# EvolBioInf/andi

Hardware: AMD Instinct MI355X
Metric: genome-pairs/sec (ordered pairs, n^2-n) over the N x N anchor-distance loop (higher is better)
Workload: dtype u8

## Files before the change

### andi_amd/csrc/esa_build.hip

```cpp
#include "andi_dev.h"
#include "esa_build.h"
#include "scan.h"
#include "knobs.h"

#include <cstring>

#define CHECK_LAUNCH()                                                                             \
	do {                                                                                           \
		hipError_t e_ = hipGetLastError();                                                         \
		if (e_ != hipSuccess) return e_;                                                           \
	} while (0)

__global__ __launch_bounds__(256) void k_phi_scatter(const int32_t *__restrict__ SA,
													 int32_t *__restrict__ phi, int32_t n) {
	int32_t r = blockIdx.x * blockDim.x + threadIdx.x;
	if (r >= n) return;
	int32_t prev = r ? SA[r - 1] : -1;
	phi[SA[r]] = prev;
}

#define PLCP_CHUNK 32
__global__ __launch_bounds__(256) void k_plcp_chunks(const uint8_t *__restrict__ S,
													 int32_t *__restrict__ phi_plcp, int32_t n) {
	int64_t chunk = (int64_t)blockIdx.x * blockDim.x + threadIdx.x;
	int64_t t0 = chunk * PLCP_CHUNK;
	if (t0 >= n) return;
	int32_t t1 = (int32_t)((t0 + PLCP_CHUNK < n) ? t0 + PLCP_CHUNK : n);
	uint32_t h = 0;
	for (int32_t t = (int32_t)t0; t < t1; ++t) {
		int32_t prev = phi_plcp[t];
		if (prev < 0) {
			phi_plcp[t] = -1;
			continue;
		}
		g_u8p a = (g_u8p)S + prev + h, b = (g_u8p)S + t + h;
		for (;;) {
			uint64_t x = ld_u64_unaligned(a) ^ ld_u64_unaligned(b);
			if (x) {
				h += (uint32_t)(__builtin_ctzll(x) >> 3);
				break;
			}
			h += 8, a += 8, b += 8;
		}
		phi_plcp[t] = (int32_t)h;
		h = h ? h - 1 : 0;
	}
}

__global__ __launch_bounds__(256) void k_lcp_fvc(const uint8_t *__restrict__ S,
												 const int32_t *__restrict__ SA,
												 const int32_t *__restrict__ plcp,
												 int32_t *__restrict__ LCP, uint8_t *__restrict__ FVC,
												 int32_t n) {
	int32_t r = blockIdx.x * blockDim.x + threadIdx.x;
	if (r > n) return;
	if (r == n) {
		LCP[n] = -1;
		return;
	}
	int32_t sa = SA[r];
	int32_t l = r ? plcp[sa] : -1;
	LCP[r] = l;
	FVC[r] = S[sa + l];
}

__global__ __launch_bounds__(256) void k_min64(const int32_t *__restrict__ in, int32_t count,
											   int32_t *__restrict__ out) {
	int64_t gid = (int64_t)blockIdx.x * blockDim.x + threadIdx.x;
	int32_t v = gid < count ? in[gid] : INT32_MAX;
	for (int off = 32; off; off >>= 1) {
		int32_t o = __shfl_xor(v, off);
		v = o < v ? o : v;
	}
	if ((threadIdx.x & 63) == 0 && gid < count) out[gid >> 6] = v;
}

__device__ __forceinline__ int32_t nearest_left_le(const MinTree &t, int32_t q, int32_t v) {
	int32_t cur = q - 1;
	int lvl = 0;
	for (;;) {
		bool found = false;
		for (;;) {
			if (t.lv[lvl][cur] <= v) {
				found = true;
				break;
			}
			if ((cur & 63) == 0) break;
			--cur;
		}
		if (found) break;
		cur = (cur >> 6) - 1;
		++lvl;
	}
	while (lvl > 0) {
		--lvl;
		cur = (cur << 6) + 63;
		while (t.lv[lvl][cur] > v) --cur;
	}
	return cur;
}

__device__ __forceinline__ int32_t nearest_right_lt(const MinTree &t, int32_t q, int32_t v) {
	int32_t cur = q + 1;
	int lvl = 0;
	for (;;) {
		bool found = false;
		for (;;) {
			if (t.lv[lvl][cur] < v) {
				found = true;
				break;
			}
			if ((cur & 63) == 63) break;
			++cur;
		}
		if (found) break;
		cur = (cur >> 6) + 1;
		++lvl;
	}
	while (lvl > 0) {
		--lvl;
		cur = cur << 6;
		while (t.lv[lvl][cur] >= v) ++cur;
	}
	return cur;
}

__global__ __launch_bounds__(256) void k_child_table(MinTree t, int32_t *__restrict__ CLD,
													 int32_t n) {
	int64_t gid = (int64_t)blockIdx.x * blockDim.x + threadIdx.x;
	if (gid >= n) return;
	int32_t q = (int32_t)gid + 1;
	const int32_t *LCP = t.lv[0];
	int32_t v = LCP[q];
	int32_t a = nearest_left_le(t, q, v);
	int32_t la = LCP[a];
	if (la == v) {
		CLD[a] = q;
		return;
	}
	int32_t b = nearest_right_lt(t, q, v);
	if (la <= LCP[b]) {
		CLD[b - 1] = q;
	} else {
		CLD[a] = q;
	}
}

__global__ __launch_bounds__(256) void k_kmer_table(EsaDev Ed, int4 *__restrict__ tab,
													int32_t *__restrict__ flags) {
	uint32_t code = blockIdx.x * blockDim.x + threadIdx.x;
	if (code >= (1u << (2 * ANDI_CACHE_K))) return;
	const EsaG E = esa_global(Ed);
	auto sym = [&](int pos) { return code_nt(code >> (2 * (ANDI_CACHE_K - 1 - pos))); };

	Ival in = esa_root(E);
	int pos = 0;
	Ival out;
	for (;;) {
		if (pos >= ANDI_CACHE_K) {
			out = in;
			break;
		}
		Ival ij = esa_child(E, in, sym(pos));
		if (ival_empty(ij)) {
			out = in;
			break;
		}
		if (ij.i == ij.j) {
			ij.l = pos + 1;
			out = ij;
			break;
		}
		if (ij.l <= pos + 1) {
			in = ij;
			++pos;
			continue;
		}
		if (ij.l >= ANDI_CACHE_K) {
			out = in;
			break;
		}
		g_u8p suf = E.S + E.SA[ij.i];
		int k = pos + 1;
		bool decided = false;
		for (; k < ij.l; ++k) {
			uint8_t e = suf[k];
			if (!is_acgt(e)) {
				out = ij;
				decided = true;
				flags[2] = 1;
				break;
			}
			if (e != sym(k)) {
				out = in;
				decided = true;
				break;
			}
		}
		if (decided) break;
		in = ij;
		pos = ij.l;
	}
	tab[code] = make_int4(out.l, out.i, out.j, out.m);
}

#define REC_V(x) ((x)&15u)
#define REC_SEP(x) (((x) >> 4) & 3u)
#define REC_CODE(x) ((x) >> 6)

__device__ __forceinline__ uint32_t suffix_rec(const uint8_t *__restrict__ N0, const int32_t *__restrict__ SA,
											   int32_t r, int K) {
	const uint32_t p = (uint32_t)SA[r];
	const uint64_t w = ld_u64_unaligned((g_u8p)N0 + (p >> 1)) >> (4 * (p & 1u));
	const uint64_t stop = (w & 0x4444444444444444ull) | (1ull << 62);
	uint32_t v = (uint32_t)__builtin_ctzll(stop) >> 2;
	uint32_t sep = 0;
	if (v < (uint32_t)K) {
		const uint32_t c = (uint32_t)(w >> (4 * v)) & 7u;
		sep = c == 4 ? 1u : (c == 5 ? 2u : 3u);
	} else {
		v = (uint32_t)K;
	}
	auto squeeze = [](uint32_t x) {
		x &= 0x33333333u;
		x = (x | (x >> 2)) & 0x0f0f0f0fu;
		x = (x | (x >> 4)) & 0x00ff00ffu;
		x = (x | (x >> 8)) & 0x0000ffffu;
		return x;
	};
	uint32_t y = __brev(squeeze((uint32_t)w) | (squeeze((uint32_t)(w >> 32)) << 16));
	y = ((y & 0x55555555u) << 1) | ((y >> 1) & 0x55555555u);
	return ((y >> (32 - 2 * K)) << 6) | (sep << 4) | v;
}

__device__ __forceinline__ uint32_t rec_lcp(uint32_t a, uint32_t b, int K) {
	uint32_t x = REC_CODE(a) ^ REC_CODE(b);
	uint32_t same = x ? (uint32_t)(__builtin_clz(x) - (32 - 2 * K)) >> 1 : (uint32_t)K;
	uint32_t va = REC_V(a), vb = REC_V(b);
	uint32_t m = va < vb ? va : vb;
	return same < m ? same : m;
}

__device__ __forceinline__ uint32_t rec_lcp_code(uint32_t code, uint32_t a, int K) {
	uint32_t x = code ^ REC_CODE(a);
	uint32_t same = x ? (uint32_t)(__builtin_clz(x) - (32 - 2 * K)) >> 1 : (uint32_t)K;
	uint32_t va = REC_V(a);
	return same < va ? same : va;
}

#ifndef PT_BLOCK
#define PT_BLOCK 256
#endif
#ifndef PT_GAPS
#define PT_GAPS 3
#endif
#define PT_TILE (PT_BLOCK * PT_GAPS)
#define PT_WORDS (PT_TILE / 64)
#define PT_RANKED 4096
__device__ __forceinline__ uint32_t wave_scan_incl(uint32_t v) {
	v += (uint32_t)__builtin_amdgcn_update_dpp(0, (int)v, 0x111, 0xf, 0xf, false);
	v += (uint32_t)__builtin_amdgcn_update_dpp(0, (int)v, 0x112, 0xf, 0xf, false);
	v += (uint32_t)__builtin_amdgcn_update_dpp(0, (int)v, 0x114, 0xf, 0xf, false);
	v += (uint32_t)__builtin_amdgcn_update_dpp(0, (int)v, 0x118, 0xf, 0xf, false);
	v += (uint32_t)__builtin_amdgcn_update_dpp(0, (int)v, 0x142, 0xa, 0xf, false);
	v += (uint32_t)__builtin_amdgcn_update_dpp(0, (int)v, 0x143, 0xc, 0xf, false);
	return v;
}

__device__ __forceinline__ uint32_t first_code(bool has, uint32_t L, int K) {
	const uint32_t v = REC_V(L), sh = 2 * ((uint32_t)K - v);
	const uint32_t c = ((REC_CODE(L) >> sh) << sh) + (v == (uint32_t)K ? 1u : 0u);
	return has ? c : 0u;
}

__device__ __forceinline__ void probe_table_block(const uint8_t *__restrict__ N0, const int32_t *__restrict__ SA,
												  const uint32_t *__restrict__ REC, const uint16_t *__restrict__ REC2, uint2 *__restrict__ deep,
												  int32_t *__restrict__ flags, int32_t n, int K, int single_ext, uint32_t block) {
	__shared__ uint32_t s_first[PT_TILE];
	__shared__ uint32_t s_absent[PT_TILE];
	__shared__ uint32_t s_h[PT_TILE + 2];
	__shared__ uint2 s_present[PT_TILE];
	__shared__ uint32_t s_rec[PT_TILE + 5];
	__shared__ uint64_t s_some[PT_WORDS];
	__shared__ uint32_t s_bits[PT_RANKED / 32];
	__shared__ uint32_t s_before[PT_RANKED / 32];
	__shared__ uint16_t s_owner[PT_TILE];

	const uint32_t r0 = block * PT_TILE;
	const uint32_t lane = threadIdx.x & 63u, wave = threadIdx.x >> 6;
	auto make_rec = [&](int32_t j) { return REC ? REC[j] : suffix_rec(N0, SA, j, K); };
	uint32_t mine2[PT_GAPS];
	{
		uint32_t mine[PT_GAPS];
#pragma unroll
		for (int u = 0; u < PT_GAPS; ++u) {
			const uint32_t g = r0 + threadIdx.x + u * PT_BLOCK;
			mine[u] = g < (uint32_t)n ? make_rec((int32_t)g) : 0u;
			mine2[u] = (single_ext == 2 && REC2 && g < (uint32_t)n) ? REC2[g] : 0u;
		}
#pragma unroll
		for (int u = 0; u < PT_GAPS; ++u) s_rec[threadIdx.x + u * PT_BLOCK + 2] = mine[u];
	}
	if (threadIdx.x < 2) s_rec[threadIdx.x] = r0 + threadIdx.x >= 2 ? make_rec((int32_t)(r0 + threadIdx.x - 2)) : 0u;
	if (threadIdx.x == 2) s_rec[PT_TILE + 2] = r0 + PT_TILE < (uint32_t)n ? make_rec((int32_t)(r0 + PT_TILE)) : 0u;
	if (threadIdx.x < PT_RANKED / 32) s_bits[threadIdx.x] = 0;
	__syncthreads();
	auto rec = [&](int32_t j) {
		const uint32_t k = (uint32_t)j - r0 + 2;
		return k < PT_TILE + 3 ? s_rec[k] : make_rec(j);
	};
	const uint32_t full = (uint32_t)K;
	if (threadIdx.x == 0) s_h[0] = r0 >= 2 ? rec_lcp(s_rec[0], s_rec[1], K) : 0u;
	if (threadIdx.x == 1) s_h[PT_TILE + 1] = r0 + PT_TILE < (uint32_t)n ? rec_lcp(s_rec[PT_TILE + 1], s_rec[PT_TILE + 2], K) : 0u;

	uint32_t counts[PT_GAPS], firsts[PT_GAPS];
#pragma unroll
	for (int u = 0; u < PT_GAPS; ++u) {
		const uint32_t i = threadIdx.x + u * PT_BLOCK;
		const uint32_t gid = r0 + i;
		const bool live = gid <= (uint32_t)n;
		const int32_t r = (int32_t)(live ? gid : 0);
		const bool hasL = live && r > 0, hasR = live && r < n;
		const uint32_t Lr = s_rec[i + 1], Rr = s_rec[i + 2], a1 = s_rec[i + 3], a2 = s_rec[i + 4], a3 = s_rec[i + 5];
		const uint32_t L = hasL ? Lr : 0u, R = hasR ? Rr : 0u;
		const uint32_t sa_r = hasR ? (uint32_t)SA[r] : 0u;
		const uint32_t h = (hasL && hasR) ? rec_lcp(L, R, K) : 0u;
		s_h[i + 1] = h;
		uint32_t absent = 0, first = 1u << (2 * K), owns_present = 0;
		uint2 present = make_uint2(0, 0);

		if (live) {
			if (hasR && REC_V(R) == full && !(hasL && L == R)) {
				const bool in_tile = i + 5 < PT_TILE + 3;
				const int32_t m = a1 != R ? 0 : (a2 != R ? 1 : (a3 != R ? 2 : 3));
				int32_t j = in_tile ? r + m : r;
				const bool more = !in_tile || m == 3;
				if (more) {
					while (j + 1 < n && j - r < 16 && rec(j + 1) == R) ++j;
					if (j - r == 16 && j + 1 < n && rec(j + 1) == R) {
						int32_t lo = j + 1, hi = n - 1;
						while (lo < hi) {
							const int32_t mid = lo + ((hi - lo + 1) >> 1);
							if (rec(mid) == R) lo = mid; else hi = mid - 1;
						}
						j = lo;
					}
				}
				if (j == r) {
					const uint32_t pos = sa_r, e0 = pos + full;
					if (single_ext == 2 && REC2) {
						const uint32_t w = mine2[u];
						present = make_uint2(pos, DEEP_SINGLE | ((w >> 8) << 2) | ((w & 0xffu) << 6));
					} else if (single_ext != 1) {
						present = make_uint2(pos, DEEP_SINGLE | (1u << 2) | (full << 8));
					} else {
						const uint64_t w = ld_u64_unaligned((g_u8p)N0 + (e0 >> 1)) >> (4 * (e0 & 1u));
						uint32_t nval = (uint32_t)__builtin_ctzll((w & 0x4444444444444444ull) | (1ull << 52)) >> 2;
						auto squeeze = [](uint32_t x) {
							x &= 0x33333333u;
							x = (x | (x >> 2)) & 0x0f0f0f0fu;
							x = (x | (x >> 4)) & 0x00ff00ffu;
							x = (x | (x >> 8)) & 0x0000ffffu;
							return x;
						};
						const uint32_t ext = (squeeze((uint32_t)w) | (squeeze((uint32_t)(w >> 32)) << 16)) & ((1u << (2 * nval)) - 1u);
						present = make_uint2(pos, DEEP_SINGLE | (nval << 2) | (ext << 6));
					}
				} else {
					const bool fits = (uint32_t)(j - r) < (1u << 24);
					present = make_uint2(fits ? (uint32_t)r : 0u, fits ? DEEP_MULTI | ((uint32_t)(j - r) << 8) : (uint32_t)DEEP_SEARCH);
				}
				owns_present = 1;
			}

			if (__builtin_amdgcn_ballot_w64(hasR && (REC_SEP(R) == 1 || REC_SEP(R) == 2)) != 0 && hasR) {
				uint32_t k = REC_V(R), sp = REC_SEP(R);
				if (k >= 1 && k <= 8 && k < full && (sp == 1 || sp == 2) && (!hasL || h < k)) {
					int32_t j = r;
					while (j + 1 < n) {
						uint32_t X = rec(j + 1);
						if (REC_V(X) == k && REC_SEP(X) == sp && rec_lcp(R, X, K) == k) ++j; else break;
					}
					if (j > r && (j + 1 == n || rec_lcp(R, rec(j + 1), K) < k)) flags[0] = 1;
				}
			}

			const int32_t lo = (int32_t)first_code(hasL, L, K);
			const uint32_t shR = 2 * (full - REC_V(R));
			const int32_t hi = hasR ? (int32_t)((REC_CODE(R) >> shR) << shR) - 1 : (int32_t)((1u << (2 * K)) - 1u);
			if (lo <= hi) absent = (uint32_t)(hi - lo + 1);
			first = (uint32_t)lo;
		}
		s_first[i] = first, s_absent[i] = absent, s_present[i] = present;
		counts[u] = absent + owns_present, firsts[u] = first;
		const uint64_t b = __ballot(counts[u] != 0);
		if (lane == 0) s_some[u * (PT_BLOCK / 64) + wave] = b;
	}

	__syncthreads();
	const uint32_t base = first_code(r0 > 0, s_rec[1], K);
	const uint32_t total = (r0 + PT_TILE <= (uint32_t)n ? first_code(true, s_rec[PT_TILE + 1], K) : (1u << (2 * K))) - base;
	uint32_t owners_before;
	{
		const uint32_t mine = lane < PT_WORDS ? (uint32_t)__builtin_popcountll(s_some[lane]) : 0u;
		owners_before = wave_scan_incl(mine) - mine;
	}
#pragma unroll
	for (int u = 0; u < PT_GAPS; ++u) {
		const uint32_t word = u * (PT_BLOCK / 64) + wave;
		const uint32_t before = (uint32_t)__builtin_amdgcn_readlane((int)owners_before, __builtin_amdgcn_readfirstlane((int)word));
		if (counts[u] == 0) continue;
		const uint32_t i = threadIdx.x + u * PT_BLOCK, off = firsts[u] - base;
		s_owner[before + (uint32_t)__builtin_popcountll(s_some[word] & ((1ull << lane) - 1ull))] = (uint16_t)i;
		if (off < PT_RANKED) atomicOr(&s_bits[off >> 5], 1u << (off & 31u));
	}
	__syncthreads();
	if (wave == 0) {
		uint32_t carry = 0;
		for (uint32_t w0 = 0; w0 < PT_RANKED / 32; w0 += 64) {
			const uint32_t mine = (uint32_t)__builtin_popcount(s_bits[w0 + lane]), incl = wave_scan_incl(mine);
			s_before[w0 + lane] = carry + incl - mine;
			carry += (uint32_t)__builtin_amdgcn_readlane((int)incl, 63);
		}
	}
	__syncthreads();

	auto write_entry = [&](uint32_t t, uint32_t a) {
		const uint32_t c = base + t;
		const bool is_present = c - s_first[a] >= s_absent[a];
		const uint2 pres = s_present[a];
		const uint32_t rr = r0 + a;
		const bool gL = rr > 0, gR = rr < (uint32_t)n;
		const uint32_t gl = s_rec[a + 1], gr = s_rec[a + 2], hll = s_h[a], hrr = s_h[a + 2];
		const uint32_t xL = rec_lcp_code(c, gl, K), xR = rec_lcp_code(c, gr, K);
		const uint32_t lL = gL ? xL : 0u, lR = gR ? xR : 0u;
		const bool left = lL > lR, right = lR > lL;
		const uint32_t l = left ? lL : lR;
		const uint32_t idx = left ? rr - 1 : (right ? rr : 0u);
		const bool alone = left ? (rr < 2 || hll < l) : (rr + 1 >= (uint32_t)n || hrr < l);
		const uint32_t uniq = ((left || right) && l != 0) ? (alone ? 1u : 0u) : (n == 1 ? 1u : 0u);
		const uint2 val = is_present ? pres : make_uint2(idx, DEEP_FINAL | (uniq << 2) | (l << 8));
		__builtin_nontemporal_store(((unsigned long long)val.y << 32) | val.x, (unsigned long long *)(deep + c));
	};
	const uint32_t ranked = total < PT_RANKED ? total : PT_RANKED;
	for (uint32_t t = threadIdx.x; t < ranked; t += PT_BLOCK) {
		const uint32_t word = t >> 5;
		write_entry(t, s_owner[s_before[word] + (uint32_t)__builtin_popcount(s_bits[word] & (0xffffffffu >> (31u - (t & 31u)))) - 1u]);
	}
	for (uint32_t t = PT_RANKED + threadIdx.x; t < total; t += PT_BLOCK) {
		const uint32_t c = base + t;
		uint32_t a = 0, b = PT_TILE;
		while (b - a > 1) {
			const uint32_t mid = (a + b) >> 1;
			if (s_first[mid] <= c) a = mid; else b = mid;
		}
		write_entry(t, a);
	}
}

__global__ __launch_bounds__(PT_BLOCK) void k_probe_table(const uint8_t *__restrict__ N0, const int32_t *__restrict__ SA,
														  const uint32_t *__restrict__ rec, const uint16_t *__restrict__ rec2, uint2 *__restrict__ deep,
														  int32_t *__restrict__ flags, int32_t n, int K, int single_ext) {
	probe_table_block(N0, SA, rec, rec2, deep, flags, n, K, single_ext, blockIdx.x);
}

__global__ __launch_bounds__(PT_BLOCK) void k_probe_table_batch(const AndiIndexBatchItem *__restrict__ items) {
	const AndiIndexBatchItem it = items[blockIdx.y];
	if ((uint64_t)blockIdx.x * PT_TILE > (uint64_t)it.n) return;
	probe_table_block(it.N0, it.SA, it.rec, it.rec2, it.deep, it.flags, it.n, it.deepK, it.single_ext, blockIdx.x);
}

size_t andi_min_tree_entries(int32_t n) {
	size_t total = 0;
	size_t cnt = (size_t)n + 1;
	while (cnt > 64) {
		cnt = (cnt + 63) / 64;
		total += cnt;
	}
	return total ? total : 1;
}

int andi_index_single_ext(size_t queries, bool sorted_on_device) {
	const int coop = andi_coop_enabled();
	if (coop == 0) return 0;
	if (const char *f = andi_knob(KNOB_SINGLE_EXT)) {
		const int v = atoi(f);
		if (v >= 0 && v <= 2 && (v != 2 || sorted_on_device)) return v;
	}
	if (sorted_on_device) return 2;
	return (coop > 0 || queries >= 256) ? 1 : 0;
}

hipError_t andi_launch_index_build(const EsaBuildArgs &a, int single_ext, hipStream_t st) {
	const int32_t n = a.n;
	hipError_t e;
	e = andi_launch_pack_symbols(a.S, (size_t)n + 1 + 64, a.N0, a.N1, a.flags + 1, st);
	if (e != hipSuccess) return e;
	if (a.P) e = andi_launch_pack_planes(a.N0, (size_t)n + 1 + 64, a.P, st);
	if (e != hipSuccess) return e;
	k_probe_table<<<(unsigned)(((int64_t)n + 1 + PT_TILE - 1) / PT_TILE), PT_BLOCK, 0, st>>>(a.N0, a.SA, a.rec, a.rec2, a.deep, a.flags, n,
																				  a.deepK, single_ext);
	CHECK_LAUNCH();
	return hipSuccess;
}

hipError_t andi_launch_index_build_batch(const AndiIndexBatchItem *d_items, uint32_t count, int32_t max_n, hipStream_t st) {
	if (count == 0) return hipSuccess;
	hipError_t e = andi_launch_pack_symbols_batch(d_items, count, (size_t)max_n + 1 + 64, st);
	if (e != hipSuccess) return e;
	e = andi_launch_pack_planes_batch(d_items, count, (size_t)max_n, st);
	if (e != hipSuccess) return e;
	const dim3 grid((unsigned)(((int64_t)max_n + 1 + PT_TILE - 1) / PT_TILE), count);
	k_probe_table_batch<<<grid, PT_BLOCK, 0, st>>>(d_items);
	CHECK_LAUNCH();
	return hipSuccess;
}

hipError_t andi_launch_esa_build(const EsaBuildArgs &a, hipStream_t st) {
	const int32_t n = a.n;
	const int B = 256;
	auto blocks = [&](int64_t items) { return (unsigned)((items + B - 1) / B); };

	int32_t *plcp = a.CLD;
	k_phi_scatter<<<blocks(n), B, 0, st>>>(a.SA, plcp, n);
	CHECK_LAUNCH();
	int64_t chunks = ((int64_t)n + PLCP_CHUNK - 1) / PLCP_CHUNK;
	k_plcp_chunks<<<blocks(chunks), B, 0, st>>>(a.S, plcp, n);
	CHECK_LAUNCH();
	k_lcp_fvc<<<blocks((int64_t)n + 1), B, 0, st>>>(a.S, a.SA, plcp, a.LCP, a.FVC, n);
	CHECK_LAUNCH();

	MinTree t;
	t.lv[0] = a.LCP;
	t.cnt[0] = n + 1;
	t.levels = 1;
	int32_t *next = a.min_scratch;
	while (t.cnt[t.levels - 1] > 64 && t.levels < ANDI_MIN_LEVELS) {
		int32_t in_cnt = t.cnt[t.levels - 1];
		int32_t out_cnt = (in_cnt + 63) / 64;
		k_min64<<<blocks(in_cnt), B, 0, st>>>(t.lv[t.levels - 1], in_cnt, next);
		CHECK_LAUNCH();
		t.lv[t.levels] = next;
		t.cnt[t.levels] = out_cnt;
		next += out_cnt;
		t.levels++;
	}
	hipError_t e = hipMemsetAsync(a.CLD, 0xff, ((size_t)n + 1) * sizeof(int32_t), st);
	if (e != hipSuccess) return e;
	k_child_table<<<blocks(n), B, 0, st>>>(t, a.CLD, n);
	CHECK_LAUNCH();

	EsaDev E;
	memset(&E, 0, sizeof E);
	E.S = a.S, E.SA = a.SA, E.LCP = a.LCP, E.CLD = a.CLD, E.FVC = a.FVC, E.tab = a.tab;
	E.flags = a.flags;
	E.n = n, E.mode = ANDI_MODE_REFERENCE;
	k_kmer_table<<<blocks(1 << (2 * ANDI_CACHE_K)), B, 0, st>>>(E, a.tab, a.flags);
	CHECK_LAUNCH();
	return hipSuccess;
}

__global__ __launch_bounds__(256) void k_rs_from_query(uint8_t *__restrict__ RS, const uint8_t *__restrict__ q, uint32_t len) {
	const uint64_t w = (uint64_t)blockIdx.x * 256 + threadIdx.x, o = 4 * w, n = 2 * (uint64_t)len + 1;
	if (o >= n) return;
	uint32_t word = 0;
#pragma unroll
	for (uint32_t k = 0; k < 4; ++k) {
		const uint64_t p = o + k;
		uint32_t c = 0;
		if (p < len) {
			c = q[len - 1 - p];
			c = c < 'A' ? (uint32_t)';' : (c ^ ((c & 2u) ? 4u : 21u));
		} else if (p == len) {
			c = '#';
		} else if (p < n) {
			c = q[p - len - 1];
		}
		word |= c << (8 * k);
	}
	((uint32_t *)RS)[w] = word;
}

#define GC_CHUNK 65536u
__global__ __launch_bounds__(256) void k_gc_counts(const uint8_t *__restrict__ pool, const uint64_t *__restrict__ off, const uint32_t *__restrict__ len,
													unsigned long long *__restrict__ counts) {
	const uint32_t qi = blockIdx.y, L = len[qi];
	const uint64_t c0 = (uint64_t)blockIdx.x * GC_CHUNK;
	if (c0 >= L) return;
	const uint8_t *s = pool + off[qi];
	const uint64_t c1 = c0 + GC_CHUNK < L ? c0 + GC_CHUNK : L;
	uint32_t cnt = 0;
	for (uint64_t p = c0 + 16ull * threadIdx.x; p < c1; p += 16ull * 256) {
		const uint4 v = *(const uint4 *)(s + p);
		const uint32_t ws[4] = {v.x, v.y, v.z, v.w};
#pragma unroll
		for (int j = 0; j < 4; ++j)
#pragma unroll
			for (int b = 0; b < 4; ++b) {
				const uint32_t c = (ws[j] >> (8 * b)) & 0xffu;
				cnt += (p + 4 * j + b < c1) && ((c & 0xfbu) == 0x43u);
			}
	}
	for (int o = 32; o > 0; o >>= 1) cnt += __shfl_down(cnt, o);
	if ((threadIdx.x & 63u) == 0 && cnt) atomicAdd(&counts[qi], (unsigned long long)cnt);
}

__global__ __launch_bounds__(256) void k_sep_counts(const uint8_t *__restrict__ pool, const uint64_t *__restrict__ off, const uint32_t *__restrict__ len,
													 uint32_t *__restrict__ counts) {
	const uint32_t qi = blockIdx.y, L = len[qi];
	const uint64_t c0 = (uint64_t)blockIdx.x * GC_CHUNK;
	if (c0 >= L) return;
	const uint8_t *s = pool + off[qi];
	const uint64_t c1 = c0 + GC_CHUNK < L ? c0 + GC_CHUNK : L;
	uint32_t cnt = 0;
	for (uint64_t p = c0 + 16ull * threadIdx.x; p < c1; p += 16ull * 256) {
		const uint4 v = *(const uint4 *)(s + p);
		const uint32_t ws[4] = {v.x, v.y, v.z, v.w};
#pragma unroll
		for (int j = 0; j < 4; ++j) {
#pragma unroll
			for (int b = 0; b < 4; ++b) cnt += (p + 4 * j + b < c1) && (((ws[j] >> (8 * b)) & 0xffu) == (uint32_t)'!');
		}
	}
	for (int o = 32; o > 0; o >>= 1) cnt += __shfl_down(cnt, o);
	if ((threadIdx.x & 63u) == 0 && cnt) atomicAdd(&counts[qi], cnt);
}

hipError_t andi_launch_sep_counts(const uint8_t *pool, const uint64_t *d_off, const uint32_t *d_len, uint32_t nq, uint32_t longest,
								  uint32_t *d_counts, hipStream_t st) {
	if (!nq || !longest) return hipSuccess;
	for (uint32_t q0 = 0; q0 < nq; q0 += 65535u) {
		const uint32_t cnt = nq - q0 < 65535u ? nq - q0 : 65535u;
		k_sep_counts<<<dim3((longest + GC_CHUNK - 1) / GC_CHUNK, cnt), 256, 0, st>>>(pool, d_off + q0, d_len + q0, d_counts + q0);
		CHECK_LAUNCH();
	}
	return hipSuccess;
}

hipError_t andi_launch_rs_from_query(uint8_t *RS, const uint8_t *q, uint32_t len, hipStream_t st) {
	const uint64_t words = (2 * (uint64_t)len + 1 + 3) / 4;
	k_rs_from_query<<<(unsigned)((words + 255) / 256), 256, 0, st>>>(RS, q, len);
	CHECK_LAUNCH();
	return hipSuccess;
}

hipError_t andi_launch_gc_counts(const uint8_t *pool, const uint64_t *d_off, const uint32_t *d_len, uint32_t nq, uint32_t longest,
								 unsigned long long *d_counts, hipStream_t st) {
	if (!nq || !longest) return hipSuccess;
	for (uint32_t q0 = 0; q0 < nq; q0 += 65535u) {
		const uint32_t cnt = nq - q0 < 65535u ? nq - q0 : 65535u;
		k_gc_counts<<<dim3((longest + GC_CHUNK - 1) / GC_CHUNK, cnt), 256, 0, st>>>(pool, d_off + q0, d_len + q0, d_counts + q0);
		CHECK_LAUNCH();
	}
	return hipSuccess;
}
```

Baseline: 137,500.

## Pack probe-table gap data into uint4 and specialize kernel on K

```diff
diff --git a/andi_amd/csrc/esa_build.hip b/andi_amd/csrc/esa_build.hip
--- a/andi_amd/csrc/esa_build.hip
+++ b/andi_amd/csrc/esa_build.hip
@@ -273,22 +273,35 @@
 	return has ? c : 0u;
 }
 
-__device__ __forceinline__ void probe_table_block(const uint8_t *__restrict__ N0, const int32_t *__restrict__ SA,
+__device__ __forceinline__ uint32_t nb_word(bool has, uint32_t rec, int K) {
+	return has ? (REC_CODE(rec) << (32 - 2 * K)) | REC_V(rec) : 0u;
+}
+
+__device__ __forceinline__ uint32_t nb_lcp(uint32_t cs, uint32_t w) {
+	const uint32_t same = (uint32_t)__builtin_clz((cs ^ w) | 1u) >> 1, v = w & 15u;
+	return same < v ? same : v;
+}
+
+struct ProbeTableShared {
+	uint4 gap[PT_TILE];
+	uint2 present[PT_TILE];
+	uint32_t rec[PT_TILE + 5];
+	uint64_t some[PT_WORDS];
+	uint32_t bits[PT_RANKED / 32];
+	uint32_t before[PT_RANKED / 32];
+	uint16_t owner[PT_TILE];
+};
+
+template <int KC, bool SE2>
+__device__ __forceinline__ void probe_table_block(ProbeTableShared &sm, const uint8_t *__restrict__ N0, const int32_t *__restrict__ SA,
 												  const uint32_t *__restrict__ REC, const uint16_t *__restrict__ REC2, uint2 *__restrict__ deep,
-												  int32_t *__restrict__ flags, int32_t n, int K, int single_ext, uint32_t block) {
-	__shared__ uint32_t s_first[PT_TILE];
-	__shared__ uint32_t s_absent[PT_TILE];
-	__shared__ uint32_t s_h[PT_TILE + 2];
-	__shared__ uint2 s_present[PT_TILE];
-	__shared__ uint32_t s_rec[PT_TILE + 5];
-	__shared__ uint64_t s_some[PT_WORDS];
-	__shared__ uint32_t s_bits[PT_RANKED / 32];
-	__shared__ uint32_t s_before[PT_RANKED / 32];
-	__shared__ uint16_t s_owner[PT_TILE];
-
+												  int32_t *__restrict__ flags, int32_t n, int Kr, int single_ext_r, uint32_t block) {
+	const int K = KC ? KC : Kr;
+	const int single_ext = SE2 ? 2 : single_ext_r;
+	const bool has_rec = SE2 || REC, short_ext = SE2 || (single_ext == 2 && REC2);
 	const uint32_t r0 = block * PT_TILE;
 	const uint32_t lane = threadIdx.x & 63u, wave = threadIdx.x >> 6;
-	auto make_rec = [&](int32_t j) { return REC ? REC[j] : suffix_rec(N0, SA, j, K); };
+	auto make_rec = [&](int32_t j) { return has_rec ? REC[j] : suffix_rec(N0, SA, j, K); };
 	uint32_t mine2[PT_GAPS];
 	{
 		uint32_t mine[PT_GAPS];
@@ -296,22 +309,20 @@
 		for (int u = 0; u < PT_GAPS; ++u) {
 			const uint32_t g = r0 + threadIdx.x + u * PT_BLOCK;
 			mine[u] = g < (uint32_t)n ? make_rec((int32_t)g) : 0u;
-			mine2[u] = (single_ext == 2 && REC2 && g < (uint32_t)n) ? REC2[g] : 0u;
-		}
-#pragma unroll
-		for (int u = 0; u < PT_GAPS; ++u) s_rec[threadIdx.x + u * PT_BLOCK + 2] = mine[u];
-	}
-	if (threadIdx.x < 2) s_rec[threadIdx.x] = r0 + threadIdx.x >= 2 ? make_rec((int32_t)(r0 + threadIdx.x - 2)) : 0u;
-	if (threadIdx.x == 2) s_rec[PT_TILE + 2] = r0 + PT_TILE < (uint32_t)n ? make_rec((int32_t)(r0 + PT_TILE)) : 0u;
-	if (threadIdx.x < PT_RANKED / 32) s_bits[threadIdx.x] = 0;
+			mine2[u] = (short_ext && g < (uint32_t)n) ? REC2[g] : 0u;
+		}
+#pragma unroll
+		for (int u = 0; u < PT_GAPS; ++u) sm.rec[threadIdx.x + u * PT_BLOCK + 2] = mine[u];
+	}
+	if (threadIdx.x < 2) sm.rec[threadIdx.x] = r0 + threadIdx.x >= 2 ? make_rec((int32_t)(r0 + threadIdx.x - 2)) : 0u;
+	if (threadIdx.x == 2) sm.rec[PT_TILE + 2] = r0 + PT_TILE < (uint32_t)n ? make_rec((int32_t)(r0 + PT_TILE)) : 0u;
+	if (threadIdx.x < PT_RANKED / 32) sm.bits[threadIdx.x] = 0;
 	__syncthreads();
 	auto rec = [&](int32_t j) {
 		const uint32_t k = (uint32_t)j - r0 + 2;
-		return k < PT_TILE + 3 ? s_rec[k] : make_rec(j);
+		return k < PT_TILE + 3 ? sm.rec[k] : make_rec(j);
 	};
 	const uint32_t full = (uint32_t)K;
-	if (threadIdx.x == 0) s_h[0] = r0 >= 2 ? rec_lcp(s_rec[0], s_rec[1], K) : 0u;
-	if (threadIdx.x == 1) s_h[PT_TILE + 1] = r0 + PT_TILE < (uint32_t)n ? rec_lcp(s_rec[PT_TILE + 1], s_rec[PT_TILE + 2], K) : 0u;
 
 	uint32_t counts[PT_GAPS], firsts[PT_GAPS];
 #pragma unroll
@@ -321,11 +332,11 @@
 		const bool live = gid <= (uint32_t)n;
 		const int32_t r = (int32_t)(live ? gid : 0);
 		const bool hasL = live && r > 0, hasR = live && r < n;
-		const uint32_t Lr = s_rec[i + 1], Rr = s_rec[i + 2], a1 = s_rec[i + 3], a2 = s_rec[i + 4], a3 = s_rec[i + 5];
+		const uint32_t Ll = sm.rec[i], Lr = sm.rec[i + 1], Rr = sm.rec[i + 2], a1 = sm.rec[i + 3], a2 = sm.rec[i + 4], a3 = sm.rec[i + 5];
 		const uint32_t L = hasL ? Lr : 0u, R = hasR ? Rr : 0u;
 		const uint32_t sa_r = hasR ? (uint32_t)SA[r] : 0u;
 		const uint32_t h = (hasL && hasR) ? rec_lcp(L, R, K) : 0u;
-		s_h[i + 1] = h;
+		const uint32_t tl = r >= 2 ? rec_lcp(Ll, Lr, K) : 0u, tr = r + 1 < n ? rec_lcp(Rr, a1, K) : 0u;
 		uint32_t absent = 0, first = 1u << (2 * K), owns_present = 0;
 		uint2 present = make_uint2(0, 0);
 
@@ -348,7 +359,7 @@
 				}
 				if (j == r) {
 					const uint32_t pos = sa_r, e0 = pos + full;
-					if (single_ext == 2 && REC2) {
+					if (short_ext) {
 						const uint32_t w = mine2[u];
 						present = make_uint2(pos, DEEP_SINGLE | ((w >> 8) << 2) | ((w & 0xffu) << 6));
 					} else if (single_ext != 1) {
@@ -391,18 +402,19 @@
 			if (lo <= hi) absent = (uint32_t)(hi - lo + 1);
 			first = (uint32_t)lo;
 		}
-		s_first[i] = first, s_absent[i] = absent, s_present[i] = present;
+		sm.gap[i] = make_uint4(first + absent, nb_word(hasL, L, K), nb_word(hasR, R, K), tl | (tr << 8));
+		sm.present[i] = present;
 		counts[u] = absent + owns_present, firsts[u] = first;
 		const uint64_t b = __ballot(counts[u] != 0);
-		if (lane == 0) s_some[u * (PT_BLOCK / 64) + wave] = b;
+		if (lane == 0) sm.some[u * (PT_BLOCK / 64) + wave] = b;
 	}
 
 	__syncthreads();
-	const uint32_t base = first_code(r0 > 0, s_rec[1], K);
-	const uint32_t total = (r0 + PT_TILE <= (uint32_t)n ? first_code(true, s_rec[PT_TILE + 1], K) : (1u << (2 * K))) - base;
+	const uint32_t base = first_code(r0 > 0, sm.rec[1], K);
+	const uint32_t total = (r0 + PT_TILE <= (uint32_t)n ? first_code(true, sm.rec[PT_TILE + 1], K) : (1u << (2 * K))) - base;
 	uint32_t owners_before;
 	{
-		const uint32_t mine = lane < PT_WORDS ? (uint32_t)__builtin_popcountll(s_some[lane]) : 0u;
+		const uint32_t mine = lane < PT_WORDS ? (uint32_t)__builtin_popcountll(sm.some[lane]) : 0u;
 		owners_before = wave_scan_incl(mine) - mine;
 	}
 #pragma unroll
@@ -411,63 +423,82 @@
 		const uint32_t before = (uint32_t)__builtin_amdgcn_readlane((int)owners_before, __builtin_amdgcn_readfirstlane((int)word));
 		if (counts[u] == 0) continue;
 		const uint32_t i = threadIdx.x + u * PT_BLOCK, off = firsts[u] - base;
-		s_owner[before + (uint32_t)__builtin_popcountll(s_some[word] & ((1ull << lane) - 1ull))] = (uint16_t)i;
-		if (off < PT_RANKED) atomicOr(&s_bits[off >> 5], 1u << (off & 31u));
+		sm.owner[before + (uint32_t)__builtin_popcountll(sm.some[word] & ((1ull << lane) - 1ull))] = (uint16_t)i;
+		if (off < PT_RANKED) atomicOr(&sm.bits[off >> 5], 1u << (off & 31u));
 	}
 	__syncthreads();
 	if (wave == 0) {
 		uint32_t carry = 0;
 		for (uint32_t w0 = 0; w0 < PT_RANKED / 32; w0 += 64) {
-			const uint32_t mine = (uint32_t)__builtin_popcount(s_bits[w0 + lane]), incl = wave_scan_incl(mine);
-			s_before[w0 + lane] = carry + incl - mine;
+			const uint32_t mine = (uint32_t)__builtin_popcount(sm.bits[w0 + lane]), incl = wave_scan_incl(mine);
+			sm.before[w0 + lane] = carry + incl - mine;
 			carry += (uint32_t)__builtin_amdgcn_readlane((int)incl, 63);
 		}
 	}
 	__syncthreads();
 
+	typedef ANDI_GLOBAL unsigned long long *g_u64p;
 	auto write_entry = [&](uint32_t t, uint32_t a) {
 		const uint32_t c = base + t;
-		const bool is_present = c - s_first[a] >= s_absent[a];
-		const uint2 pres = s_present[a];
-		const uint32_t rr = r0 + a;
-		const bool gL = rr > 0, gR = rr < (uint32_t)n;
-		const uint32_t gl = s_rec[a + 1], gr = s_rec[a + 2], hll = s_h[a], hrr = s_h[a + 2];
-		const uint32_t xL = rec_lcp_code(c, gl, K), xR = rec_lcp_code(c, gr, K);
-		const uint32_t lL = gL ? xL : 0u, lR = gR ? xR : 0u;
+		const uint4 g = sm.gap[a];
+		const uint32_t cs = c << (32 - 2 * K), lL = nb_lcp(cs, g.y), lR = nb_lcp(cs, g.z);
 		const bool left = lL > lR, right = lR > lL;
-		const uint32_t l = left ? lL : lR;
+		const uint32_t l = left ? lL : lR, rr = r0 + a;
 		const uint32_t idx = left ? rr - 1 : (right ? rr : 0u);
-		const bool alone = left ? (rr < 2 || hll < l) : (rr + 1 >= (uint32_t)n || hrr < l);
-		const uint32_t uniq = ((left || right) && l != 0) ? (alone ? 1u : 0u) : (n == 1 ? 1u : 0u);
-		const uint2 val = is_present ? pres : make_uint2(idx, DEEP_FINAL | (uniq << 2) | (l << 8));
-		__builtin_nontemporal_store(((unsigned long long)val.y << 32) | val.x, (unsigned long long *)(deep + c));
+		const uint32_t thr = left ? g.w & 0xffu : g.w >> 8;
+		const uint32_t uniq = (left || right) ? (thr < l ? 1u : 0u) : (n == 1 ? 1u : 0u);
+		uint2 val = make_uint2(idx, DEEP_FINAL | (uniq << 2) | (l << 8));
+		if (c >= g.x) val = sm.present[a];
+		__builtin_nontemporal_store(((unsigned long long)val.y << 32) | val.x, (g_u64p)(deep + c));
 	};
 	const uint32_t ranked = total < PT_RANKED ? total : PT_RANKED;
 	for (uint32_t t = threadIdx.x; t < ranked; t += PT_BLOCK) {
 		const uint32_t word = t >> 5;
-		write_entry(t, s_owner[s_before[word] + (uint32_t)__builtin_popcount(s_bits[word] & (0xffffffffu >> (31u - (t & 31u)))) - 1u]);
-	}
+		write_entry(t, sm.owner[sm.before[word] + (uint32_t)__builtin_popcount(sm.bits[word] & (0xffffffffu >> (31u - (t & 31u)))) - 1u]);
+	}
+	auto first_of = [&](uint32_t m) {
+		const uint32_t gid = r0 + m;
+		return gid <= (uint32_t)n ? first_code(gid > 0, sm.rec[m + 1], K) : (1u << (2 * K));
+	};
 	for (uint32_t t = PT_RANKED + threadIdx.x; t < total; t += PT_BLOCK) {
 		const uint32_t c = base + t;
 		uint32_t a = 0, b = PT_TILE;
 		while (b - a > 1) {
 			const uint32_t mid = (a + b) >> 1;
-			if (s_first[mid] <= c) a = mid; else b = mid;
+			if (first_of(mid) <= c) a = mid; else b = mid;
 		}
 		write_entry(t, a);
 	}
+}
+
+__device__ __forceinline__ void probe_table_any(ProbeTableShared &sm, const uint8_t *N0, const int32_t *SA, const uint32_t *REC,
+												const uint16_t *REC2, uint2 *deep, int32_t *flags, int32_t n, int K, int single_ext, uint32_t block) {
+#define PT_CALL(KC, SE2) probe_table_block<KC, SE2>(sm, N0, SA, REC, REC2, deep, flags, n, K, single_ext, block)
+	const bool se2 = REC && REC2 && single_ext == 2;
+#ifdef PT_ONE_INSTANCE
+	PT_CALL(0, false); return;
+#endif
+	switch (K) {
+	case 11: if (se2) PT_CALL(11, true); else PT_CALL(11, false); break;
+	case 12: if (se2) PT_CALL(12, true); else PT_CALL(12, false); break;
+	case 13: if (se2) PT_CALL(13, true); else PT_CALL(13, false); break;
+	default: if (se2) PT_CALL(0, true); else PT_CALL(0, false); break;
+	}
+#undef PT_CALL
 }
 
 __global__ __launch_bounds__(PT_BLOCK) void k_probe_table(const uint8_t *__restrict__ N0, const int32_t *__restrict__ SA,
 														  const uint32_t *__restrict__ rec, const uint16_t *__restrict__ rec2, uint2 *__restrict__ deep,
 														  int32_t *__restrict__ flags, int32_t n, int K, int single_ext) {
-	probe_table_block(N0, SA, rec, rec2, deep, flags, n, K, single_ext, blockIdx.x);
+	__shared__ ProbeTableShared sm;
+	probe_table_any(sm, N0, SA, rec, rec2, deep, flags, n, K, single_ext, blockIdx.x);
 }
 
 __global__ __launch_bounds__(PT_BLOCK) void k_probe_table_batch(const AndiIndexBatchItem *__restrict__ items) {
+	__shared__ ProbeTableShared sm;
 	const AndiIndexBatchItem it = items[blockIdx.y];
 	if ((uint64_t)blockIdx.x * PT_TILE > (uint64_t)it.n) return;
-	probe_table_block(it.N0, it.SA, it.rec, it.rec2, it.deep, it.flags, it.n, it.deepK, it.single_ext, blockIdx.x);
+	probe_table_any(sm, it.N0, it.SA, it.rec, it.rec2, it.deep, it.flags, it.n, it.deepK, it.single_ext, blockIdx.x);
 }
 
 size_t andi_min_tree_entries(int32_t n) {
```

Result: no change. 135,100, median of 6 (-1.7%).
